# LemonATsu/UNet-PhaseGen

Measured on AMD Instinct MI355X. Metric: spectrogram-frames/sec (train fwd+bwd), higher is better.
Workload: dtype f32; 1 GPU; train.py full step (fwd + cos/sin/mag loss + bwd + Adam), UNetModel(1024, 2048), per-GPU batch 64 x 1024 bins x 256 frames (BASELINE configs[2]); global_batch=64, frames=256, channels=1024, parallelism=dp1, grad_allreduce_payload=fp32, adam=fused into the wgrad epilogues

## Files before the change

include/phasegen.h:

```cpp
#ifndef PHASEGEN_H
#define PHASEGEN_H
#include <stdint.h>

#ifdef __cplusplus
extern "C" {
#endif

#define PG_VERSION 400

enum { PG_OK = 0, PG_ERR_NULL = -1, PG_ERR_SHAPE = -2, PG_ERR_ALIGN = -3, PG_ERR_UNSUPPORTED = -4,
       PG_ERR_WORKSPACE = -5 };

enum { PG_ACT_NONE = 0, PG_ACT_LEAKY02 = 1 , PG_ACT_RELU = 2  };

struct pg_adam_args;
typedef struct pg_conv_args {
    int32_t B, Cin, Cout, Lin, Lout, k, stride, pad;
    const float* x;  int64_t x_bs;
    int32_t x_act;
    int32_t precision;
    const float* w;
    float* y;        int64_t y_bs;
    const float* dy; int64_t dy_bs;
    float* dx;       int64_t dx_bs;
    const float* dx_add; int64_t dx_add_bs;
    const float* dx_ref; int64_t dx_ref_bs;
    int32_t dx_mask;
    int32_t schedule;
    float* dw;
    int32_t y_act; int32_t y2_act;
    float* y2;       int64_t y2_bs;
    void* workspace; int64_t workspace_bytes;
    const struct pg_adam_args* adam;
} pg_conv_args;
int64_t pg_workspace_bytes_conv(void);
int64_t pg_workspace_bytes_wgrad(const pg_conv_args* a, int32_t op);
enum { PG_PREC_FP32 = 0, PG_PREC_BF16 = 1, PG_PREC_BF16X3 = 2 };
enum { PG_SCHED_AUTO = 0, PG_SCHED_TILE_PER_WG = 1, PG_SCHED_FORCE_STREAMK = 2, PG_SCHED_NO_RAW = 4, PG_SCHED_NO_TALL = 8,
       PG_SCHED_CONTENDED = 16, PG_SCHED_NO_PS = 128, PG_SCHED_NO_RAW3 = 0x2000, PG_SCHED_ALL_RAW3 = 0x4000, PG_SCHED_NO_COLSPLIT = 0x20000, PG_SCHED_COLSPLIT = 0x40000 };
#define PG_SCHED_OVERSUB(f) (((f) & 15) << 8)
#define PG_SCHED_SLOTS(n) (((n) & 31) << 19)

int pg_conv1d_fwd(const pg_conv_args* a, void* stream);
int pg_conv1d_dgrad(const pg_conv_args* a, void* stream);
int pg_conv1d_wgrad(const pg_conv_args* a, void* stream);
int pg_convt1d_fwd(const pg_conv_args* a, void* stream);
int pg_convt1d_dgrad(const pg_conv_args* a, void* stream);
int pg_convt1d_wgrad(const pg_conv_args* a, void* stream);
enum { PG_OP_CONV1D_FWD = 0, PG_OP_CONV1D_DGRAD = 1, PG_OP_CONV1D_WGRAD = 2,
       PG_OP_CONVT1D_FWD = 3, PG_OP_CONVT1D_DGRAD = 4, PG_OP_CONVT1D_WGRAD = 5 };
int pg_conv_describe(const pg_conv_args* a, int32_t op, char* buf, int32_t buflen);

#define PG_H_HEAD 32
typedef struct pg_convh_args {
// ... 238 lines not shown
```

unet-phasegen_amd/csrc/conv_common.h:

```cpp
#pragma once
#include <hip/hip_runtime.h>
#include <stdint.h>
#include "phasegen.h"
#include "pg_common.h"

namespace pgconv {

struct IgemmParams {
    const float* x; long x_bs;
    const float* w;
    const float* pt; long pt_bs;
    float* y; long y_bs;
    const float* add; long add_bs;
    const float* ref; long ref_bs;
    unsigned x_bytes, w_bytes, pt_bytes;
    int B, Q, M, Lx, Ly, k, s, p;
    int act_x, act_p, mask_mode;
    int U, u_off;
    int LP; float inv_LP;
    int a_vec;
    int tilesM, tilesN;
    int g_ps;
    int tn_stride;
    float* y2; long y2_bs; float y_slope, y2_slope;
// ... 439 lines not shown
constexpr int RS2 = 768, RS1 = 384;
constexpr int raw_gap(int tj) { return tj >= 8 ? 16 : tj; }
constexpr int RTILE_A = RBM * BK;
constexpr int g_wlp(int kw, int s) { return kw == 32 ? 64 : (kw == 8 ? (s == 1 ? 24 : 40) : 36); }

inline bool unet_ks(int k, int s) { return (k == 32 && s == 2) || (k == 8 && s == 1) || (k == 8 && s == 2) || (k == 4 && s == 2) || (k == 5 && s == 2); }

enum Kind { KIND_F, KIND_T, KIND_G };

}

namespace pgconv {
hipError_t launch_im2col(int kind, const IgemmParams& p, int grid, hipStream_t st, int prec);
hipError_t launch_raw_ft(int kind, const IgemmParams& p, int grid, hipStream_t st, int prec);
hipError_t launch_raw_ft_tall(int kind, const IgemmParams& p, int grid, hipStream_t st, int prec);
hipError_t launch_raw_g(const IgemmParams& p, int grid, hipStream_t st, int prec);
hipError_t launch_h3(int kind, const IgemmParams& p, int grid, hipStream_t st);
bool raw3_covers(int kind, const IgemmParams& p);
hipError_t launch_raw3(int kind, const IgemmParams& p, int grid, hipStream_t st);
bool h_supported(int kind, const IgemmParams& p);
}
```

unet-phasegen_amd/csrc/conv_igemm.hip:

```cpp
#include <hip/hip_runtime.h>
#include <cstring>
#include <cmath>
#include <algorithm>
#include "conv_fixup.h"

namespace {

constexpr int WG_PER_CU = 2;
constexpr int MAX_STREAMK_WG = 2048;
constexpr long WS_PER_WG = 2L * ACC_REGS * NT * 4;
constexpr long WS_STREAMK = (long)MAX_STREAMK_WG * WS_PER_WG;

struct Knobs {
    int prec;
    int force_mode;
    int no_raw;
    int no_tall;
    int oversub;
    int contended;
    int no_ps;
    int no_raw3;
    int all_raw3;
    int sr;
    int force_colsplit;
    int no_colsplit;
    int slots;
};
int decode_knobs(const pg_conv_args* a, Knobs& k) {
    if (a->precision < 0 || a->precision > 2) return pg_fail(PG_ERR_UNSUPPORTED, "conv: precision must be PG_PREC_FP32, PG_PREC_BF16 or PG_PREC_BF16X3");
    const int sc = a->schedule;
    if (sc < 0 || (sc & ~0xffffff) || ((sc >> 17) & 3) == 3 || (sc & 3) == 3 || ((sc >> 8) & 15) > 8) return pg_fail(PG_ERR_SHAPE, "conv: bad schedule bits");
    k.prec = a->precision;
    k.force_mode = sc & 3; k.no_raw = (sc >> 2) & 1; k.no_tall = (sc >> 3) & 1;
    k.oversub = (sc >> 8) & 15; if (!k.oversub) k.oversub = 4;
    k.contended = (sc >> 4) & 1;
    if ((sc >> 5) & 3) return pg_fail(PG_ERR_UNSUPPORTED, "conv: schedule bits 5-6 (tile families removed in 0.4)");
    k.no_ps = (sc >> 7) & 1;
    k.no_raw3 = (sc >> 13) & 1;
    k.all_raw3 = (sc >> 14) & 1;
    k.sr = ((sc >> 15) & 3) ? 1 << (((sc >> 15) & 3) - 1) : 0;
    k.no_colsplit = (sc >> 17) & 1;
    k.force_colsplit = (sc >> 18) & 1;
    k.slots = (sc >> 19) & 31;
    if (k.no_raw3 && k.all_raw3) return pg_fail(PG_ERR_SHAPE, "conv: schedule bits 13 and 14 exclude each other");
    return PG_OK;
}

bool fixup_wide(int grid, long split_tiles) { return split_tiles > 0 && grid >= 8 * split_tiles; }

int pick_grid(long tiles, int nslab, IgemmParams& p, long ws_bytes, const Knobs& kn, bool one_wave) {
    const long total = tiles * (long)nslab;
    const long slots = (long)(kn.slots ? kn.slots : pg_cu_count()) * (one_wave ? 1 : WG_PER_CU), ws_per_wg = one_wave ? 2 * WS_PER_WG : WS_PER_WG;
    ws_bytes = std::min(ws_bytes, WS_STREAMK);
    p.whole = 0;
    if (kn.force_mode == 0 && !kn.contended && tiles % slots == 0) {
        if (tiles <= slots * kn.oversub) return (int)tiles;
        for (long mult = kn.oversub; mult >= 1; --mult)
            if (tiles % (slots * mult) == 0) return (int)(slots * mult);
    }
// ... 39 lines not shown
    p.Kp = (int)kp; p.pk_bytes = (unsigned)pbytes;
    return (qbytes + 255) / 256 * 256 + pbytes;
}

enum Family { FAM_IM2COL, FAM_RAW, FAM_RAW_TALL, FAM_RAW3, FAM_G_RAW, FAM_G_PS, FAM_H3 };
enum Fixup { FIXUP_NONE, FIXUP_PLAIN, FIXUP_WIDE };
struct ConvPart {
    Family fam; int grid; long tiles; Fixup fixup;
    IgemmParams p;
};
struct ConvPlan {
    Kind kind; int prec;
    ConvPart main, tail;
    bool has_tail;
    long pack;
};

bool r3_ok(Kind kind, const IgemmParams& p, const Knobs& kn, long rows) {
    return kind != KIND_G && kn.prec == 0 && !kn.no_raw3 && raw_supported(kind, p, kn) && pgconv::raw3_covers(kind, p) &&
           (rows + 255) / 256 * 256 * 100 <= (rows + RBM - 1) / RBM * RBM * 103;
}

Family pick_family(Kind kind, const IgemmParams& p, const Knobs& kn, long rows, long cols) {
    const bool raw = raw_supported(kind, p, kn);
    if (kind == KIND_G) {
        if (!raw) return FAM_IM2COL;
        const long cps = (p.LP + 15) / 16;
        return p.k != 32 && (cps * 16 - p.LP) * 100 <= 7L * p.LP && !kn.no_ps ? FAM_G_PS : FAM_G_RAW;
    }
    const long cols_wide = (cols + RBN - 1) / RBN * RBN, cols_tall = (cols + RBN / 2 - 1) / (RBN / 2) * (RBN / 2);
// ... 92 lines not shown
    return PG_OK;
}

struct ConvOp { Kind kind; bool tr, swap; const char* null_msg; };
const ConvOp CONV_OPS[6] = {
    {KIND_F, false, false, "conv1d_fwd: x, w, y required"},
    {KIND_T, false, true, "conv1d_dgrad: dy, w, dx required"},
    {KIND_G, false, false, "conv1d_wgrad: dy, x, dw required"},
    {KIND_T, true, false, "convt1d_fwd: x, w, y required"},
    {KIND_F, true, true, "convt1d_dgrad: dy, w, dx required"},
    {KIND_G, true, true, "convt1d_wgrad: dy, x, dw required"}};

int plan_conv(int op, const pg_conv_args* a, bool ptrs, ConvPlan& pl) {
    const ConvOp& o = CONV_OPS[op];
    if (int e = check_geom(a, o.tr)) return e;
    Knobs kn; if (int e = decode_knobs(a, kn)) return e;
    IgemmParams p = {};
    p.B = a->B; p.k = a->k; p.s = a->stride; p.p = a->pad;
    p.M = o.swap ? a->Cin : a->Cout; p.Q = o.swap ? a->Cout : a->Cin; p.Lx = o.swap ? a->Lout : a->Lin;
    const int lo = o.swap ? a->Lin : a->Lout;
    p.x = o.swap ? a->dy : a->x; p.x_bs = o.swap ? a->dy_bs : a->x_bs; p.act_x = o.swap ? PG_ACT_NONE : a->x_act;
    if (o.kind == KIND_G) {
        p.pt = o.swap ? a->x : a->dy; p.pt_bs = o.swap ? a->x_bs : a->dy_bs; p.act_p = o.swap ? a->x_act : PG_ACT_NONE;
        p.LP = lo; p.y = a->dw;
    } else if (o.swap) {
        p.w = a->w; p.Ly = lo; p.y = a->dx; p.y_bs = a->dx_bs; p.y_slope = 1.0f; p.y2_slope = 1.0f;
        p.add = a->dx_add; p.add_bs = a->dx_add_bs; p.ref = a->dx_ref; p.ref_bs = a->dx_ref_bs;
        p.mask_mode = a->dx_ref ? a->dx_mask : 0;
    } else {
        p.w = a->w; p.Ly = lo; p.y = a->y; p.y_bs = a->y_bs; p.y_slope = pg_act_slope(a->y_act);
        p.y2 = a->y2; p.y2_bs = a->y2_bs; p.y2_slope = pg_act_slope(a->y2_act);
    }
    if (ptrs && (!p.x || !p.y || !(o.kind == KIND_G ? p.pt : p.w))) return pg_fail(PG_ERR_NULL, o.null_msg);
    long rows = p.M, cols = (long)p.B * p.Ly, K = (long)p.Q * p.k;
    if (o.kind == KIND_T) {
        p.u_off = p.p / p.s;
        p.U = (p.Ly - 1 + p.p) / p.s - p.u_off + 1;
        if (p.U <= 0) return pg_fail(PG_ERR_SHAPE, "convT: empty output");
        rows = (long)p.M * p.s; cols = (long)p.B * p.U; K = (long)p.Q * ((p.k + p.s - 1) / p.s);
    } else if (o.kind == KIND_G) {
        cols = (long)p.Q * p.k; K = (long)p.B * p.LP;
    }
    if (int e = set_extents(p)) return e;
    if (int e = o.kind == KIND_G ? set_fused_adam(p, a) : PG_OK) return e;
    p.ws = (float*)a->workspace;
    pl.kind = o.kind; pl.prec = kn.prec; pl.pack = 0;
    pl.has_tail = split_columns(o.kind, p, kn, rows, cols, K, a->workspace_bytes);
    if (pl.has_tail) {
        const long full = cols / RBN * RBN;
        if (int e = plan_part(FAM_RAW3, o.kind, kn, p, rows, 0, full, K, a->workspace_bytes, pl.main)) return e;
        return plan_part(FAM_RAW_TALL, o.kind, kn, p, rows, full, cols, K, a->workspace_bytes, pl.tail);
    }
    const Family fam = pick_family(o.kind, p, kn, rows, cols);
    if (int e = plan_part(fam, o.kind, kn, p, rows, 0, cols, K, a->workspace_bytes, pl.main)) return e;
    if ((pl.main.fam == FAM_G_RAW || pl.main.fam == FAM_G_PS) && kn.prec == 0 && (pl.pack = g_pack_layout(pl.main.p)) < 0)
        return pg_fail(PG_ERR_SHAPE, "wgrad: packed operand exceeds 2 GiB (31-bit buffer offsets)");
    return PG_OK;
}

int h3_params(const pg_convh_args* a, bool ptrs, IgemmParams& p, Knobs& kn) {
    if (!a) return pg_fail(PG_ERR_NULL, "conv_fwd_h: null args");
// ... 28 lines not shown
    if (tr) {
        p.u_off = p.p / p.s;
        p.U = (p.Ly - 1 + p.p) / p.s - p.u_off + 1;
        if (p.U <= 0) return pg_fail(PG_ERR_SHAPE, "conv_fwd_h: empty output");
    }
    if (!pgconv::h_supported(tr ? KIND_T : KIND_F, p)) return pg_fail(PG_ERR_UNSUPPORTED, "conv_fwd_h: geometry not covered by the bf16-resident kernels (use the fp32-tensor entry points)");
    return PG_OK;
}

int plan_h3(const pg_convh_args* a, ConvPlan& pl) {
    Knobs kn;
    ConvPart& c = pl.main;
    IgemmParams& p = c.p;
    if (int e = h3_params(a, true, p, kn)) return e;
    const bool tr = a->transposed != 0;
    pl.kind = tr ? KIND_T : KIND_F; pl.prec = 0; pl.has_tail = false; pl.pack = 0; c.fam = FAM_H3;
    const long rows = tr ? (long)p.M * p.s : p.M, cols = (long)p.B * (tr ? p.U : p.Ly);
    p.tilesM = (int)((rows + 255) / 256);
    p.tilesN = (int)((cols + 255) / 256);
    p.tn_stride = 256;
    p.nslab = (int)((long)p.Q * (tr ? pg_shadow_taps(p.k, p.s) : p.k) / 32);
    c.tiles = (long)p.tilesM * p.tilesN;
    if (c.tiles <= 0 || c.tiles > 0x0fffffffL || p.nslab <= 0) return pg_fail(PG_ERR_SHAPE, "conv_fwd_h: empty or oversize grid");
    set_grid(c, kn, a->workspace_bytes);
    return PG_OK;
}

hipError_t launch_fixup(const ConvPlan& pl, const ConvPart& c, hipStream_t st) {
    typedef void (*Fn)(const IgemmParams, int);
#define FIX2(KIND, MB, NB, WN) {conv_fixup_kernel<KIND, MB, NB, WN, false>, conv_fixup_kernel<KIND, MB, NB, WN, true>}
    static const Fn table[4][4][2] = {
// ... 17 lines not shown
    const Kind kind = pl.kind;
    const char* tk = kind == KIND_T ? "true" : "false";
    hipError_t e = hipSuccess;
    switch (c.fam) {
        case FAM_RAW_TALL:
            if (name) snprintf(name, 96, "conv_raw_kernel<%d, %d, %s, %d, 1>", p.k, p.s, tk, pl.prec);
            else e = pgconv::launch_raw_ft_tall(kind, p, c.grid, st, pl.prec);
            break;
        case FAM_RAW:
            if (name) snprintf(name, 96, "conv_raw_kernel<%d, %d, %s, %d, 2>", p.k, p.s, tk, pl.prec);
            else e = pgconv::launch_raw_ft(kind, p, c.grid, st, pl.prec);
            break;
        case FAM_G_RAW:
        case FAM_G_PS:
            if (name) snprintf(name, 96, "conv_g_%s_kernel<%d, %d, %d>", c.fam == FAM_G_PS ? "ps" : "raw", p.k, p.s, pl.prec);
            else e = pgconv::launch_raw_g(p, c.grid, st, pl.prec);
            break;
        case FAM_IM2COL:
            if (name) snprintf(name, 96, "conv_%c_kernel<0, 0, %d>", "ftg"[kind], pl.prec);
            else e = pgconv::launch_im2col(kind, p, c.grid, st, pl.prec);
            break;
        case FAM_RAW3:
            if (name) snprintf(name, 96, "conv_raw3_kernel<%d, %d, %s, %s>", p.k, p.s, tk, p.act_x == PG_ACT_NONE ? "false" : "true");
            else e = pgconv::launch_raw3(kind, p, c.grid, st);
            break;
        case FAM_H3:
            if (name) snprintf(name, 96, "conv_h3_kernel<%d, %d, %s>", kind == KIND_T && p.k == 5 ? 8 : p.k, p.s, tk);
            else e = pgconv::launch_h3(kind, p, c.grid, st);
            break;
    }
    if (!name && e == hipSuccess && c.fixup != FIXUP_NONE) e = launch_fixup(pl, c, st);
    return e;
}

void describe(const ConvPlan& pl, char* buf, int buflen) {
    static const char* const fixup_name[] = {"none", "plain", "wide"};
    const ConvPart& c = pl.main;
    char name[96];
    (void)part_kernel(pl, c, nullptr, name);
    snprintf(buf, (size_t)buflen, "%s|grid=%d|tiles=%ld|slabs=%d|split=%d|whole=%d|fixup=%s", name, c.grid, c.tiles, c.p.nslab,
             (int)(c.fixup != FIXUP_NONE), c.p.whole, fixup_name[c.fixup]);
    if (!pl.has_tail) return;
    (void)part_kernel(pl, pl.tail, nullptr, name);
    const size_t n = strlen(buf);
    if (n + 7 < (size_t)buflen) snprintf(buf + n, (size_t)buflen - n, "|tail=%s,grid=%d", name, pl.tail.grid);
}

int execute(ConvPlan& pl, long ws_bytes, hipStream_t st) {
    IgemmParams& p = pl.main.p;
    if (pl.pack) {
        if (!p.ws || ws_bytes < WS_STREAMK + pl.pack)
            return pg_fail(PG_ERR_WORKSPACE, "wgrad: the fp32 kernels need pg_workspace_bytes_wgrad() bytes of workspace (packed operands)");
        p.qk = reinterpret_cast<const float*>(reinterpret_cast<char*>(p.ws) + WS_STREAMK);
        p.pk = reinterpret_cast<const float*>(reinterpret_cast<const char*>(p.qk) + ((long)p.qk_bytes + 255) / 256 * 256);
    }
    hipError_t e = part_kernel(pl, pl.main, st);
    if (e == hipSuccess && pl.has_tail) e = part_kernel(pl, pl.tail, st);
    return e == hipSuccess ? PG_OK : pg_fail((int)e, hipGetErrorString(e));
}

int run_conv(int op, const pg_conv_args* a, void* stream) {
    ConvPlan pl;
    if (int e = plan_conv(op, a, true, pl)) return e;
    return execute(pl, a->workspace_bytes, (hipStream_t)stream);
}

}

extern "C" int pg_conv1d_fwd(const pg_conv_args* a, void* stream) { return run_conv(PG_OP_CONV1D_FWD, a, stream); }
// ... 43 lines not shown
```

unet-phasegen_amd/csrc/conv_raw_wgrad.hip:

```cpp
#include "conv_common.h"

namespace {

template <int KW, int S> struct GRaw {
    static constexpr int WL = 15 * S + KW;
    static constexpr int WLP = g_wlp(KW, S);
    static constexpr int NQT = RBN / KW;
    static constexpr int TNV = NQT * KW;
    static constexpr int SUB = NQT * WLP;
    static constexpr int SUBS = (SUB + 63) / 64 * 64;
    static constexpr int NE = (SUB + NT - 1) / NT;
    static constexpr int STG = RTILE_A + 2 * SUBS;
    static constexpr int SUBP = (SUB + 255) / 256 * 256;
    static_assert(WL <= WLP, "window does not fit its slot");
};

template <int KW, int S, int BF>
__device__ __forceinline__ void g_raw_bf(const IgemmParams& p) {
    using C = GRaw<KW, S>;
    __shared__ __attribute__((aligned(16))) float lds[2 * C::STG];
    const int tid = threadIdx.x, lane = tid & 63;
    const int wv = __builtin_amdgcn_readfirstlane(tid >> 6), wm = wv >> 1, wn = wv & 1;
    const int kt = dma_kt(lane, wv);
    const rsrc_t rp = make_rsrc(p.pt, p.pt_bytes), rx = make_rsrc(p.x, p.x_bytes);
// ... 568 lines not shown
        slot = 1;
    }
}

template <int KW, int S, int BF>
__global__ __launch_bounds__(NT, 2) void conv_g_raw_kernel(const IgemmParams p) {
    if constexpr (BF == 0) g_raw_f32<KW, S>(p);
    else g_raw_bf<KW, S, BF>(p);
}
template <int KW, int S, int BF>
__global__ __launch_bounds__(NT, 2) void conv_g_ps_kernel(const IgemmParams p) {
    if constexpr (BF == 0) g_ps_f32<KW, S>(p);
    else g_ps_bf<KW, S, BF>(p);
}

__global__ __launch_bounds__(256) void pack_rows_kernel(const float* __restrict__ src, long bs, int C, int L, int F, int W, unsigned n,
                                                       float slope, float* __restrict__ dst) {
    for (unsigned i = blockIdx.x * 256u + threadIdx.x; i < n; i += gridDim.x * 256u) {
        const unsigned r = i / (unsigned)W, b = r / (unsigned)C, c = r - b * (unsigned)C;
        const int t = (int)(i - r * (unsigned)W) - F;
        float v = 0.f;
        if ((unsigned)t < (unsigned)L) {
            v = src[(long)b * bs + (long)c * L + t];
            if (slope != 1.0f) v = pg_act_apply(v, slope);
        }
        dst[i] = v;
    }
}
__global__ __launch_bounds__(256) void pack_flat_kernel(const float* __restrict__ src, long bs, int B, int LP, int Kp, unsigned n,
                                                       float slope, float* __restrict__ dst) {
    for (unsigned i = blockIdx.x * 256u + threadIdx.x; i < n; i += gridDim.x * 256u) {
        const unsigned m = i / (unsigned)Kp, k = i - m * (unsigned)Kp, b = k / (unsigned)LP, t = k - b * (unsigned)LP;
        float v = 0.f;
        if ((int)b < B) {
            v = src[(long)b * bs + (long)m * LP + t];
            if (slope != 1.0f) v = pg_act_apply(v, slope);
        }
        dst[i] = v;
    }
}
unsigned pack_grid(unsigned n) { return (n + 255u) / 256u < 2048u ? (n + 255u) / 256u : 2048u; }

hipError_t pack_g(const IgemmParams& p, hipStream_t st) {
    float* const qk = const_cast<float*>(p.qk);
    float* const pk = const_cast<float*>(p.pk);
    const unsigned nq = (unsigned)(p.qk_bytes / 4), np = (unsigned)(p.pk_bytes / 4);
    hipLaunchKernelGGL(pack_rows_kernel, dim3(pack_grid(nq)), dim3(256), 0, st, p.x, p.x_bs, p.Q, p.Lx, p.p, p.Lq, nq, pg_act_slope(p.act_x), qk);
    if (p.g_ps) hipLaunchKernelGGL(pack_rows_kernel, dim3(pack_grid(np)), dim3(256), 0, st, p.pt, p.pt_bs, p.M, p.LP, 0, p.Kp, np, pg_act_slope(p.act_p), pk);
    else hipLaunchKernelGGL(pack_flat_kernel, dim3(pack_grid(np)), dim3(256), 0, st, p.pt, p.pt_bs, p.B, p.LP, p.Kp, np, pg_act_slope(p.act_p), pk);
    return hipGetLastError();
}

template <int KW, int S>
hipError_t launch_g_raw(const IgemmParams& p, int grid, hipStream_t st, int prec) {
    if (prec == 0) {
        if (hipError_t e = pack_g(p, st)) return e;
    }
    if (p.g_ps) {
        if (prec == 1) hipLaunchKernelGGL((conv_g_ps_kernel<KW, S, 1>), dim3(grid), dim3(NT), 0, st, p);
        else if (prec == 2) hipLaunchKernelGGL((conv_g_ps_kernel<KW, S, 2>), dim3(grid), dim3(NT), 0, st, p);
        else hipLaunchKernelGGL((conv_g_ps_kernel<KW, S, 0>), dim3(grid), dim3(NT), 0, st, p);
        return hipGetLastError();
    }
    if (prec == 1) hipLaunchKernelGGL((conv_g_raw_kernel<KW, S, 1>), dim3(grid), dim3(NT), 0, st, p);
    else if (prec == 2) hipLaunchKernelGGL((conv_g_raw_kernel<KW, S, 2>), dim3(grid), dim3(NT), 0, st, p);
    else hipLaunchKernelGGL((conv_g_raw_kernel<KW, S, 0>), dim3(grid), dim3(NT), 0, st, p);
    return hipGetLastError();
}

}

hipError_t pgconv::launch_raw_g(const IgemmParams& p, int grid, hipStream_t st, int prec) {
    if (p.k == 32) return launch_g_raw<32, 2>(p, grid, st, prec);
    if (p.k == 8 && p.s == 1) return launch_g_raw<8, 1>(p, grid, st, prec);
    if (p.k == 8) return launch_g_raw<8, 2>(p, grid, st, prec);
    if (p.k == 5) return launch_g_raw<5, 2>(p, grid, st, prec);
    return launch_g_raw<4, 2>(p, grid, st, prec);
}
```

unet-phasegen_amd/phasegen/_lib.py:

```python
import ctypes as C
import os

_HERE = os.path.dirname(os.path.abspath(__file__))
LIB_PATH = os.path.join(_HERE, "libphasegen.so")
ABI_VERSION = 400

ACT_NONE, ACT_LEAKY, ACT_RELU = 0, 1, 2
PREC_FP32, PREC_BF16, PREC_BF16X3 = 0, 1, 2
OK, ERR_NULL, ERR_SHAPE, ERR_ALIGN, ERR_UNSUPPORTED, ERR_WORKSPACE = 0, -1, -2, -3, -4, -5
OP_CONV1D_FWD, OP_CONV1D_DGRAD, OP_CONV1D_WGRAD, OP_CONVT1D_FWD, OP_CONVT1D_DGRAD, OP_CONVT1D_WGRAD = range(6)
SCHED_AUTO, SCHED_TILE_PER_WG, SCHED_FORCE_STREAMK, SCHED_NO_RAW, SCHED_NO_TALL, SCHED_CONTENDED = 0, 1, 2, 4, 8, 16
SCHED_NO_PS = 128
SCHED_NO_RAW3 = 0x2000
SCHED_ALL_RAW3 = 0x4000
SCHED_NO_COLSPLIT = 0x20000
SCHED_COLSPLIT = 0x40000


def SCHED_SLOTS(n):
    if not 0 <= n <= 31:
        raise ValueError("SCHED_SLOTS: n must be 0..31")
    return n << 19


RS_KAISER_BEST, RS_KAISER_FAST = 0, 1

c_float_p = C.c_void_p


class ConvArgs(C.Structure):
    _fields_ = [("B", C.c_int32), ("Cin", C.c_int32), ("Cout", C.c_int32), ("Lin", C.c_int32), ("Lout", C.c_int32),
# ... 259 lines not shown
```

unet-phasegen_amd/phasegen/ops.py:

```python
import contextlib
import ctypes as C
import threading

import torch

from . import _lib
from ._lib import ACT_LEAKY, ACT_NONE, ACT_RELU, SCHED_CONTENDED, SCHED_SLOTS, SCHED_TILE_PER_WG


def _stream():
    return C.c_void_p(torch.cuda.current_stream().cuda_stream)


def _on_current_device(t, name):
    if t.device.index != torch.cuda.current_device():
        raise ValueError(f"{name}: tensor is on {t.device} but the current device is cuda:{torch.cuda.current_device()} "
                         "(wrap the call in torch.cuda.device(...))")


class KernelTimer:

    def __init__(self):
        self.records = {}
        self.plans = {}
# ... 106 lines not shown
    def clear(self):
        self.d.clear()


_conv_ws = _StreamCache()
_caches = [_conv_ws]


def _workspace(cache, device, need, what):
    if need < 0:
        _lib.check(int(need), what)
    ws = cache.get(device, lambda: need, need)
    return ws.data_ptr(), ws.numel()


def conv_workspace(device):
    return _conv_ws.get(device, _lib.load().pg_workspace_bytes_conv)


def release_workspaces():
    for c in _caches:
        c.clear()


_PRECISIONS = {"fp32": 0, "f32": 0, "bf16": 1, "bf16x3": 2, 0: 0, 1: 1, 2: 2}


class _Defaults(threading.local):
    precision = 0
    schedule = 0
    stft_single = 0


_tls = _Defaults()


def precision_code(mode):
    if mode not in _PRECISIONS:
        raise ValueError(f"conv precision {mode!r}: expected fp32 / bf16 / bf16x3 (or 0 / 1 / 2)")
    return _PRECISIONS[mode]


def set_conv_precision(mode):
    _tls.precision = precision_code(mode)


def current_schedule():
    return _tls.schedule


def set_conv_schedule(mode):
    if mode < 0 or (mode & ~0xffe0ff) or (mode & 0x60000) == 0x60000 or (mode & 3) == 3 or (mode & 0x70) or (mode & 0x6000) == 0x6000:
        raise ValueError("conv schedule: bad mode")
    _tls.schedule = (_tls.schedule & 0xf00) | mode


def set_conv_oversubscribe(factor):
    if not 1 <= factor <= 8:
        raise ValueError("conv oversubscribe: factor must be 1..8")
# ... 77 lines not shown
    lib = _lib.load()
    _note_plan(a, _lib.OP_CONVT1D_DGRAD if transposed else _lib.OP_CONV1D_DGRAD)
    fn = lib.pg_convt1d_dgrad if transposed else lib.pg_conv1d_dgrad
    _lib.check(fn(C.byref(a), _stream()), "dgrad")
    return dx


def adam_args(p, m, v, step, lr=1e-3, beta1=0.9, beta2=0.999, eps=1e-8, grad_scale=1.0):
    a = _lib.AdamArgs()
    a.n = p.numel()
    a.p, a.m, a.v = _dense(p, "p"), _dense(m, "m"), _dense(v, "v")
    a.lr, a.beta1, a.beta2, a.eps, a.grad_scale, a.step = lr, beta1, beta2, eps, grad_scale, step
    return a


def conv_wgrad(x, dy, dw, stride, pad, x_act=ACT_NONE, transposed=False, precision=None, schedule=None, adam=None):
    Cin, Cout, k = _geom(transposed, dw.shape)
    B, _, Lin = x.shape
    a = _conv_args(transposed, B, Cin, Cout, Lin, k, stride, pad, x.device, precision, schedule)
    if tuple(x.shape) != (B, Cin, Lin) or tuple(dy.shape) != (B, Cout, a.Lout):
        raise ValueError(f"conv_wgrad: shapes x{tuple(x.shape)} dy{tuple(dy.shape)} dw{tuple(dw.shape)} inconsistent")
    a.x, a.x_bs = _act3(x, "x")
    a.dy, a.dy_bs = _act3(dy, "dy")
    a.dw = _dense(dw, "dw")
    a.x_act = x_act
    if adam is not None:
        if adam.n != dw.numel():
            raise ValueError("conv_wgrad: fused adam tensors must have dw's shape")
        a.adam = C.addressof(adam)
    lib = _lib.load()
    op = _lib.OP_CONVT1D_WGRAD if transposed else _lib.OP_CONV1D_WGRAD
    need = lib.pg_workspace_bytes_wgrad(C.byref(a), op)
    if need > a.workspace_bytes:
        ws = _conv_ws.get(x.device, lib.pg_workspace_bytes_conv, at_least=need)
        a.workspace, a.workspace_bytes = ws.data_ptr(), ws.numel()
    _note_plan(a, op)
    fn = lib.pg_convt1d_wgrad if transposed else lib.pg_conv1d_wgrad
    _lib.check(fn(C.byref(a), _stream()), "wgrad")
    return dw


H_HEAD = 32
H_TAIL = 40


def h_pitch(L):
    return (L + H_TAIL + 7) // 8 * 8
# ... 766 lines not shown
```

unet-phasegen_amd/phasegen/unet.py:

```python
import math

import numpy as np
import torch

from . import detgen, ops
from .ops import ACT_LEAKY, ACT_NONE, ACT_RELU

ALIGN = 64

LAYERS = {
    "D0": (detgen.K_D0, "c", 2, 16), "D1": (detgen.K_D1, "c", 1, 2), "D2": (detgen.K_D2, "c", 2, 1),
    "D3": (detgen.K_D3, "c", 2, 1), "U3": (detgen.K_U3, "t", 2, 1), "U2": (detgen.K_U2, "t", 2, 1),
    "U1": (detgen.K_U1, "t", 1, 2), "U0": (detgen.K_U0, "t", 2, 16),
}
BN_OF = {"D1": detgen.BN_D1, "D2": detgen.BN_D2, "U3": detgen.BN_U3, "U2": detgen.BN_U2, "U1": detgen.BN_U1,
         "U0": detgen.BN_U0}
BACKWARD_ORDER = ["U0", "U1", "U2", "U3", "D3", "D2", "D1", "D0"]

CONTENDED_DGRAD = {"U0": ops.SCHED_CONTENDED, "U1": ops.SCHED_CONTENDED, "U2": ops.SCHED_CONTENDED, "U3": 0,
                   "D3": 0, "D2": ops.SCHED_CONTENDED, "D1": ops.SCHED_CONTENDED}
CONTENDED_WGRAD = {name: ops.SCHED_TILE_PER_WG for name in BACKWARD_ORDER}


def frame_plan(L):
# ... 74 lines not shown
                self.buffers[k].copy_(torch.as_tensor(np.asarray(params[k])))


class UNetEngine:

    def __init__(self, C, device=None, precision=None):
        if not torch.cuda.is_available():
            raise RuntimeError("phasegen.UNetEngine needs an MI355X (no CPU fallback exists for the hot path)")
        self.C = C
        self.device = torch.device("cuda", torch.cuda.current_device()) if device is None else torch.device(device)
        if self.device.index is None:
            self.device = torch.device("cuda", torch.cuda.current_device())
        self.precision = None if precision is None else ops.precision_code(precision)
        self.graphs = False
        self.contended = False
        self.fwd_count = 0
        self.arena = ParamArena(C, self.device)
        self.plans = {}
        self.bn_save = {k: (torch.empty(2 * C, device=self.device), torch.empty(2 * C, device=self.device))
                        for k in BN_OF}
        self.cur = None

    def plan(self, B, L):
        key = (B, L)
        if key not in self.plans:
            C = self.C
            L1, L2, L3, L4 = frame_plan(L)
            dev = self.device

            def z(*s):
# ... 210 lines not shown
        f = plan["fwd"]
        B = x0.shape[0]
        g = self._bwd_bufs(plan, B)
        a = self.arena
        h = 2 * self.C
        g_out = g_out.contiguous()
        def sched(table, name):
            return (ops.current_schedule() | table[name]) if self.contended else None

        def bn_bwd(name, raw, dy, dx):
            key = BN_OF[name]
            sm, si = self.bn_save[name]
            with ops.timed("hbm:bn_bwd." + name, 12 * raw.numel()):
                ops.bn_bwd(raw, dy, dx, a.p(key + ".weight"), sm, si, a.g(key + ".weight"), a.g(key + ".bias"))

        def wgrad(name, x, dy, act):
            key, kind, s, p = LAYERS[name]
            adam = fused_adam(key) if fused_adam is not None else None
            with ops.timed(name + ".wgrad"):
                ops.conv_wgrad(x, dy, a.g(key), s, p, x_act=act, transposed=(kind == "t"), precision=self.precision,
                               schedule=sched(CONTENDED_WGRAD, name), adam=adam)

        def dgrad(name, dy, dx, **kw):
            key, kind, s, p = LAYERS[name]
            with ops.timed(name + ".dgrad"):
                ops.conv_dgrad(dy, a.p(key), dx, s, p, transposed=(kind == "t"), precision=self.precision,
                               schedule=sched(CONTENDED_DGRAD, name), **kw)

        def ready(name):
            if on_grads_ready is not None:
                on_grads_ready(name)

        def done(name):
            if on_layer_done is not None:
                on_layer_done(name)

        def layer(name, wg, dg=None, **dkw):
            if fused_adam is None:
                wgrad(name, *wg)
                ready(name)
                if dg is not None:
                    dgrad(name, *dg, **dkw)
            else:
                if dg is not None:
                    dgrad(name, *dg, **dkw)
                wgrad(name, *wg)
                ready(name)
            done(name)

        for name, cat, raw, gin, g_raw, g_cat in (("U0", "cat0", "r0", g_out, "g_r0", "g_cat0"),
                                                  ("U1", "cat1", "r1", g["g_cat0"][:, h:], "g_r1", "g_cat1"),
                                                  ("U2", "cat2", "r2", g["g_cat1"][:, h:], "g_r2", "g_cat2"),
                                                  ("U3", "d3", "r3", g["g_cat2"][:, h:], "g_r3", "g_d3")):
            bn_bwd(name, f[raw], gin, g[g_raw])
            layer(name, (f[cat], g[g_raw], ACT_NONE), (g[g_raw], g[g_cat]), ref=f[cat], mask=ACT_RELU)
        layer("D3", (f["l2"], g["g_d3"], ACT_NONE), (g["g_d3"], g["g_cat2"][:, :h]), add=g["g_cat2"][:, :h], ref=f["l2"], mask=ACT_LEAKY)
        bn_bwd("D2", f["c2"], g["g_cat2"][:, :h], g["g_c2"])
        layer("D2", (f["l1"], g["g_c2"], ACT_NONE), (g["g_c2"], g["g_cat1"][:, :h]), add=g["g_cat1"][:, :h], ref=f["l1"], mask=ACT_LEAKY)
        bn_bwd("D1", f["c1"], g["g_cat1"][:, :h], g["g_c1"])
        layer("D1", (f["l0"], g["g_c1"], ACT_NONE), (g["g_c1"], g["g_cat0"][:, :h]), add=g["g_cat0"][:, :h], ref=f["l0"], mask=ACT_LEAKY)
        layer("D0", (x0, g["g_cat0"][:, :h], ACT_NONE))
# ... 16 lines not shown
```

Before: 99020 frames/s.

## Split fp32 wgrad operand packing into a stage that can overlap dgrad on a side stream

Replaces the separate scalar pack_rows/pack_flat kernels with one fused pack kernel that handles both operands with one wave per row unit and 16-byte vector loads and stores. Adds schedule bits to run only the pack or only the GEMM of the fp32 wgrad, plus an opt-in UNet path that packs on a side stream while dgrad runs, synchronised with events. The aim is to cut pack launch and bandwidth overhead and to hide packing behind dgrad. In exchange, the overlap needs a shared workspace sized for the largest layer, and the two streams now compete for bandwidth.

```diff
diff --git a/include/phasegen.h b/include/phasegen.h
--- a/include/phasegen.h
+++ b/include/phasegen.h
@@ -37,7 +37,8 @@
 int64_t pg_workspace_bytes_wgrad(const pg_conv_args* a, int32_t op);
 enum { PG_PREC_FP32 = 0, PG_PREC_BF16 = 1, PG_PREC_BF16X3 = 2 };
 enum { PG_SCHED_AUTO = 0, PG_SCHED_TILE_PER_WG = 1, PG_SCHED_FORCE_STREAMK = 2, PG_SCHED_NO_RAW = 4, PG_SCHED_NO_TALL = 8,
-       PG_SCHED_CONTENDED = 16, PG_SCHED_NO_PS = 128, PG_SCHED_NO_RAW3 = 0x2000, PG_SCHED_ALL_RAW3 = 0x4000, PG_SCHED_NO_COLSPLIT = 0x20000, PG_SCHED_COLSPLIT = 0x40000 };
+       PG_SCHED_CONTENDED = 16, PG_SCHED_NO_PS = 128, PG_SCHED_NO_RAW3 = 0x2000, PG_SCHED_ALL_RAW3 = 0x4000, PG_SCHED_NO_COLSPLIT = 0x20000, PG_SCHED_COLSPLIT = 0x40000,
+       PG_SCHED_PACK_ONLY = 0x1000000, PG_SCHED_PACKED = 0x2000000 };
 #define PG_SCHED_OVERSUB(f) (((f) & 15) << 8)
 #define PG_SCHED_SLOTS(n) (((n) & 31) << 19)
 
diff --git a/unet-phasegen_amd/csrc/conv_common.h b/unet-phasegen_amd/csrc/conv_common.h
--- a/unet-phasegen_amd/csrc/conv_common.h
+++ b/unet-phasegen_amd/csrc/conv_common.h
@@ -477,7 +477,8 @@
 hipError_t launch_im2col(int kind, const IgemmParams& p, int grid, hipStream_t st, int prec);
 hipError_t launch_raw_ft(int kind, const IgemmParams& p, int grid, hipStream_t st, int prec);
 hipError_t launch_raw_ft_tall(int kind, const IgemmParams& p, int grid, hipStream_t st, int prec);
-hipError_t launch_raw_g(const IgemmParams& p, int grid, hipStream_t st, int prec);
+enum { PACK_BOTH = 0, PACK_ONLY = 1, PACK_CALLER = 2 };
+hipError_t launch_raw_g(const IgemmParams& p, int grid, hipStream_t st, int prec, int pack_mode);
 hipError_t launch_h3(int kind, const IgemmParams& p, int grid, hipStream_t st);
 bool raw3_covers(int kind, const IgemmParams& p);
 hipError_t launch_raw3(int kind, const IgemmParams& p, int grid, hipStream_t st);
diff --git a/unet-phasegen_amd/csrc/conv_igemm.hip b/unet-phasegen_amd/csrc/conv_igemm.hip
--- a/unet-phasegen_amd/csrc/conv_igemm.hip
+++ b/unet-phasegen_amd/csrc/conv_igemm.hip
@@ -25,11 +25,12 @@
     int force_colsplit;
     int no_colsplit;
     int slots;
+    int pack_mode;
 };
-int decode_knobs(const pg_conv_args* a, Knobs& k) {
+int decode_knobs(const pg_conv_args* a, Knobs& k, bool wgrad = false) {
     if (a->precision < 0 || a->precision > 2) return pg_fail(PG_ERR_UNSUPPORTED, "conv: precision must be PG_PREC_FP32, PG_PREC_BF16 or PG_PREC_BF16X3");
     const int sc = a->schedule;
-    if (sc < 0 || (sc & ~0xffffff) || ((sc >> 17) & 3) == 3 || (sc & 3) == 3 || ((sc >> 8) & 15) > 8) return pg_fail(PG_ERR_SHAPE, "conv: bad schedule bits");
+    if (sc < 0 || (sc & ~(wgrad ? 0x3ffffff : 0xffffff)) || ((sc >> 17) & 3) == 3 || (sc & 3) == 3 || ((sc >> 8) & 15) > 8) return pg_fail(PG_ERR_SHAPE, "conv: bad schedule bits");
     k.prec = a->precision;
     k.force_mode = sc & 3; k.no_raw = (sc >> 2) & 1; k.no_tall = (sc >> 3) & 1;
     k.oversub = (sc >> 8) & 15; if (!k.oversub) k.oversub = 4;
@@ -43,6 +44,8 @@
     k.force_colsplit = (sc >> 18) & 1;
     k.slots = (sc >> 19) & 31;
     if (k.no_raw3 && k.all_raw3) return pg_fail(PG_ERR_SHAPE, "conv: schedule bits 13 and 14 exclude each other");
+    if ((sc & PG_SCHED_PACK_ONLY) && (sc & PG_SCHED_PACKED)) return pg_fail(PG_ERR_UNSUPPORTED, "conv: PG_SCHED_PACK_ONLY and PG_SCHED_PACKED exclude each other");
+    k.pack_mode = (sc & PG_SCHED_PACK_ONLY) ? pgconv::PACK_ONLY : ((sc & PG_SCHED_PACKED) ? pgconv::PACK_CALLER : pgconv::PACK_BOTH);
     return PG_OK;
 }
 
@@ -112,6 +115,7 @@
     ConvPart main, tail;
     bool has_tail;
     long pack;
+    int pack_mode;
 };
 
 bool r3_ok(Kind kind, const IgemmParams& p, const Knobs& kn, long rows) {
@@ -234,7 +238,7 @@
 int plan_conv(int op, const pg_conv_args* a, bool ptrs, ConvPlan& pl) {
     const ConvOp& o = CONV_OPS[op];
     if (int e = check_geom(a, o.tr)) return e;
-    Knobs kn; if (int e = decode_knobs(a, kn)) return e;
+    Knobs kn; if (int e = decode_knobs(a, kn, o.kind == KIND_G)) return e;
     IgemmParams p = {};
     p.B = a->B; p.k = a->k; p.s = a->stride; p.p = a->pad;
     p.M = o.swap ? a->Cin : a->Cout; p.Q = o.swap ? a->Cout : a->Cin; p.Lx = o.swap ? a->Lout : a->Lin;
@@ -265,6 +269,7 @@
     if (int e = o.kind == KIND_G ? set_fused_adam(p, a) : PG_OK) return e;
     p.ws = (float*)a->workspace;
     pl.kind = o.kind; pl.prec = kn.prec; pl.pack = 0;
+    pl.pack_mode = o.kind == KIND_G ? kn.pack_mode : pgconv::PACK_BOTH;
     pl.has_tail = split_columns(o.kind, p, kn, rows, cols, K, a->workspace_bytes);
     if (pl.has_tail) {
         const long full = cols / RBN * RBN;
@@ -323,7 +328,7 @@
     IgemmParams& p = c.p;
     if (int e = h3_params(a, true, p, kn)) return e;
     const bool tr = a->transposed != 0;
-    pl.kind = tr ? KIND_T : KIND_F; pl.prec = 0; pl.has_tail = false; pl.pack = 0; c.fam = FAM_H3;
+    pl.kind = tr ? KIND_T : KIND_F; pl.prec = 0; pl.has_tail = false; pl.pack = 0; pl.pack_mode = pgconv::PACK_BOTH; c.fam = FAM_H3;
     const long rows = tr ? (long)p.M * p.s : p.M, cols = (long)p.B * (tr ? p.U : p.Ly);
     p.tilesM = (int)((rows + 255) / 256);
     p.tilesN = (int)((cols + 255) / 256);
@@ -371,7 +376,7 @@
         case FAM_G_RAW:
         case FAM_G_PS:
             if (name) snprintf(name, 96, "conv_g_%s_kernel<%d, %d, %d>", c.fam == FAM_G_PS ? "ps" : "raw", p.k, p.s, pl.prec);
-            else e = pgconv::launch_raw_g(p, c.grid, st, pl.prec);
+            else e = pgconv::launch_raw_g(p, c.grid, st, pl.prec, pl.pack_mode);
             break;
         case FAM_IM2COL:
             if (name) snprintf(name, 96, "conv_%c_kernel<0, 0, %d>", "ftg"[kind], pl.prec);
@@ -397,6 +402,10 @@
     (void)part_kernel(pl, c, nullptr, name);
     snprintf(buf, (size_t)buflen, "%s|grid=%d|tiles=%ld|slabs=%d|split=%d|whole=%d|fixup=%s", name, c.grid, c.tiles, c.p.nslab,
              (int)(c.fixup != FIXUP_NONE), c.p.whole, fixup_name[c.fixup]);
+    if (pl.pack_mode != pgconv::PACK_BOTH) {
+        const size_t n = strlen(buf);
+        if (n + 13 < (size_t)buflen) snprintf(buf + n, (size_t)buflen - n, "|pack=%s", pl.pack_mode == pgconv::PACK_ONLY ? "only" : "caller");
+    }
     if (!pl.has_tail) return;
     (void)part_kernel(pl, pl.tail, nullptr, name);
     const size_t n = strlen(buf);
@@ -405,11 +414,16 @@
 
 int execute(ConvPlan& pl, long ws_bytes, hipStream_t st) {
     IgemmParams& p = pl.main.p;
+    if (pl.pack_mode == pgconv::PACK_ONLY && !pl.pack) return PG_OK;
     if (pl.pack) {
         if (!p.ws || ws_bytes < WS_STREAMK + pl.pack)
             return pg_fail(PG_ERR_WORKSPACE, "wgrad: the fp32 kernels need pg_workspace_bytes_wgrad() bytes of workspace (packed operands)");
         p.qk = reinterpret_cast<const float*>(reinterpret_cast<char*>(p.ws) + WS_STREAMK);
         p.pk = reinterpret_cast<const float*>(reinterpret_cast<const char*>(p.qk) + ((long)p.qk_bytes + 255) / 256 * 256);
+    }
+    if (pl.pack_mode == pgconv::PACK_ONLY) {
+        const hipError_t e = pgconv::launch_raw_g(p, 0, st, pl.prec, pl.pack_mode);
+        return e == hipSuccess ? PG_OK : pg_fail((int)e, hipGetErrorString(e));
     }
     hipError_t e = part_kernel(pl, pl.main, st);
     if (e == hipSuccess && pl.has_tail) e = part_kernel(pl, pl.tail, st);
diff --git a/unet-phasegen_amd/csrc/conv_raw_wgrad.hip b/unet-phasegen_amd/csrc/conv_raw_wgrad.hip
--- a/unet-phasegen_amd/csrc/conv_raw_wgrad.hip
+++ b/unet-phasegen_amd/csrc/conv_raw_wgrad.hip
@@ -606,48 +606,119 @@
     else g_ps_bf<KW, S, BF>(p);
 }
 
-__global__ __launch_bounds__(256) void pack_rows_kernel(const float* __restrict__ src, long bs, int C, int L, int F, int W, unsigned n,
-                                                       float slope, float* __restrict__ dst) {
-    for (unsigned i = blockIdx.x * 256u + threadIdx.x; i < n; i += gridDim.x * 256u) {
-        const unsigned r = i / (unsigned)W, b = r / (unsigned)C, c = r - b * (unsigned)C;
-        const int t = (int)(i - r * (unsigned)W) - F;
-        float v = 0.f;
-        if ((unsigned)t < (unsigned)L) {
-            v = src[(long)b * bs + (long)c * L + t];
-            if (slope != 1.0f) v = pg_act_apply(v, slope);
-        }
-        dst[i] = v;
-    }
-}
-__global__ __launch_bounds__(256) void pack_flat_kernel(const float* __restrict__ src, long bs, int B, int LP, int Kp, unsigned n,
-                                                       float slope, float* __restrict__ dst) {
-    for (unsigned i = blockIdx.x * 256u + threadIdx.x; i < n; i += gridDim.x * 256u) {
-        const unsigned m = i / (unsigned)Kp, k = i - m * (unsigned)Kp, b = k / (unsigned)LP, t = k - b * (unsigned)LP;
-        float v = 0.f;
-        if ((int)b < B) {
-            v = src[(long)b * bs + (long)m * LP + t];
-            if (slope != 1.0f) v = pg_act_apply(v, slope);
-        }
-        dst[i] = v;
-    }
-}
-unsigned pack_grid(unsigned n) { return (n + 255u) / 256u < 2048u ? (n + 255u) / 256u : 2048u; }
+struct PackRows {
+    const float* src; float* dst; long bs; int nrow, C, L, F, W, rw, segs; float inv_nch, slope;
+};
+struct PackFlat {
+    const float* src; float* dst; long bs; int M, B, LP, Kp, rw, segs; float inv_nch, inv_LP, slope;
+};
+struct PackUnit {
+    int r0, nr, ch0, n;
+    __device__ __forceinline__ PackUnit(unsigned u, int rows, int nch, int rw, int segs) {
+        if (segs > 1) { r0 = (int)(u / (unsigned)segs); nr = 1; ch0 = ((int)u - r0 * segs) * 256; n = min(256, nch - ch0); }
+        else { r0 = (int)u * rw; nr = min(rw, rows - r0); ch0 = 0; n = nch; }
+    }
+    __device__ __forceinline__ void piece(int idx, int nch, float inv_nch, int& q, int& ch) const {
+        if (nr == 1) { q = 0; ch = ch0 + idx; }
+        else divmod24(idx, nch, inv_nch, q, ch);
+    }
+};
+__device__ __forceinline__ f32x4 pack_load4(const float* __restrict__ sp, int t, int L) {
+    f32x4 v = {0.f, 0.f, 0.f, 0.f};
+    if (t >= 0 && t + 4 <= L) {
+        __builtin_memcpy(&v, sp + t, 16);
+    } else {
+#pragma unroll
+        for (int e = 0; e < 4; ++e)
+            if ((unsigned)(t + e) < (unsigned)L) v[e] = sp[t + e];
+    }
+    return v;
+}
+__device__ __forceinline__ void pack_store4(float* __restrict__ dp, f32x4 v, float slope) {
+    if (slope != 1.0f) {
+#pragma unroll
+        for (int e = 0; e < 4; ++e) v[e] = pg_act_apply(v[e], slope);
+    }
+    *reinterpret_cast<f32x4*>(dp) = v;
+}
+__device__ __forceinline__ void pack_rows(const PackRows& o, unsigned gw, unsigned nw, int lane) {
+    const int nch = o.W >> 2;
+    const unsigned nunits = o.segs > 1 ? (unsigned)o.nrow * o.segs : ((unsigned)o.nrow + o.rw - 1) / o.rw;
+    for (unsigned u = gw; u < nunits; u += nw) {
+        const PackUnit un(u, o.nrow, nch, o.rw, o.segs);
+        const int b0 = un.r0 / o.C, c0 = un.r0 - b0 * o.C;
+        for (int idx = lane; idx < un.nr * un.n; idx += 64) {
+            int q, ch;
+            un.piece(idx, nch, o.inv_nch, q, ch);
+            int b = b0, c = c0 + q;
+            if (c >= o.C) { c -= o.C; ++b; }
+            const float* const sp = o.src + (long)b * o.bs + (long)c * o.L;
+            pack_store4(o.dst + (long)(un.r0 + q) * o.W + 4 * ch, pack_load4(sp, 4 * ch - o.F, o.L), o.slope);
+        }
+    }
+}
+__device__ __forceinline__ void pack_flat(const PackFlat& o, unsigned gw, unsigned nw, int lane) {
+    const int nch = o.Kp >> 2, K = o.B * o.LP;
+    const unsigned nunits = o.segs > 1 ? (unsigned)o.M * o.segs : ((unsigned)o.M + o.rw - 1) / o.rw;
+    for (unsigned u = gw; u < nunits; u += nw) {
+        const PackUnit un(u, o.M, nch, o.rw, o.segs);
+        for (int idx = lane; idx < un.nr * un.n; idx += 64) {
+            int q, ch;
+            un.piece(idx, nch, o.inv_nch, q, ch);
+            const int m = un.r0 + q, k0 = 4 * ch;
+            f32x4 v = {0.f, 0.f, 0.f, 0.f};
+            if (k0 < K) {
+                int b, i0;
+                if (K < (1 << 24)) divmod24(k0, o.LP, o.inv_LP, b, i0);
+                else { b = k0 / o.LP; i0 = k0 - b * o.LP; }
+                const float* const sp = o.src + (long)b * o.bs + (long)m * o.LP;
+                v = pack_load4(sp, i0, o.LP);
+                if (i0 + 4 > o.LP && b + 1 < o.B) {
+                    const float* const sn = sp + o.bs;
+#pragma unroll
+                    for (int e = 1; e < 4; ++e)
+                        if (i0 + e >= o.LP) v[e] = sn[i0 + e - o.LP];
+                }
+            }
+            pack_store4(o.dst + (long)m * o.Kp + k0, v, o.slope);
+        }
+    }
+}
+__global__ __launch_bounds__(256) void pack_g_kernel(const PackRows q, const PackRows pr, const PackFlat pf) {
+    const int lane = threadIdx.x & 63;
+    const unsigned gw = blockIdx.x * 4u + (threadIdx.x >> 6), nw = gridDim.x * 4u;
+    pack_rows(q, gw, nw, lane);
+    if (pr.nrow) pack_rows(pr, gw, nw, lane);
+    if (pf.M) pack_flat(pf, gw, nw, lane);
+}
+void pack_units(int nch, int cap, int& rw, int& segs, long& units, long rows) {
+    segs = nch > 256 ? (nch + 255) / 256 : 1;
+    rw = segs > 1 ? 1 : std::max(1, std::min(std::min(256 / nch, 64), cap));
+    units = segs > 1 ? rows * segs : (rows + rw - 1) / rw;
+}
 
 hipError_t pack_g(const IgemmParams& p, hipStream_t st) {
     float* const qk = const_cast<float*>(p.qk);
     float* const pk = const_cast<float*>(p.pk);
-    const unsigned nq = (unsigned)(p.qk_bytes / 4), np = (unsigned)(p.pk_bytes / 4);
-    hipLaunchKernelGGL(pack_rows_kernel, dim3(pack_grid(nq)), dim3(256), 0, st, p.x, p.x_bs, p.Q, p.Lx, p.p, p.Lq, nq, pg_act_slope(p.act_x), qk);
-    if (p.g_ps) hipLaunchKernelGGL(pack_rows_kernel, dim3(pack_grid(np)), dim3(256), 0, st, p.pt, p.pt_bs, p.M, p.LP, 0, p.Kp, np, pg_act_slope(p.act_p), pk);
-    else hipLaunchKernelGGL(pack_flat_kernel, dim3(pack_grid(np)), dim3(256), 0, st, p.pt, p.pt_bs, p.B, p.LP, p.Kp, np, pg_act_slope(p.act_p), pk);
+    PackRows q = {p.x, qk, p.x_bs, p.B * p.Q, p.Q, p.Lx, p.p, p.Lq, 1, 1, 4.0f / (float)p.Lq, pg_act_slope(p.act_x)};
+    PackRows pr = {};
+    PackFlat pf = {};
+    long uq, up;
+    pack_units(p.Lq / 4, p.Q, q.rw, q.segs, uq, q.nrow);
+    if (p.g_ps) {
+        pr = {p.pt, pk, p.pt_bs, p.B * p.M, p.M, p.LP, 0, p.Kp, 1, 1, 4.0f / (float)p.Kp, pg_act_slope(p.act_p)};
+        pack_units(p.Kp / 4, p.M, pr.rw, pr.segs, up, pr.nrow);
+    } else {
+        pf = {p.pt, pk, p.pt_bs, p.M, p.B, p.LP, p.Kp, 1, 1, 4.0f / (float)p.Kp, 1.0f / (float)p.LP, pg_act_slope(p.act_p)};
+        pack_units(p.Kp / 4, p.M, pf.rw, pf.segs, up, pf.M);
+    }
+    const long wg = (std::max(uq, up) + 3) / 4;
+    hipLaunchKernelGGL(pack_g_kernel, dim3((unsigned)std::min(wg, 2048L)), dim3(256), 0, st, q, pr, pf);
     return hipGetLastError();
 }
 
 template <int KW, int S>
 hipError_t launch_g_raw(const IgemmParams& p, int grid, hipStream_t st, int prec) {
-    if (prec == 0) {
-        if (hipError_t e = pack_g(p, st)) return e;
-    }
     if (p.g_ps) {
         if (prec == 1) hipLaunchKernelGGL((conv_g_ps_kernel<KW, S, 1>), dim3(grid), dim3(NT), 0, st, p);
         else if (prec == 2) hipLaunchKernelGGL((conv_g_ps_kernel<KW, S, 2>), dim3(grid), dim3(NT), 0, st, p);
@@ -662,7 +733,11 @@
 
 }
 
-hipError_t pgconv::launch_raw_g(const IgemmParams& p, int grid, hipStream_t st, int prec) {
+hipError_t pgconv::launch_raw_g(const IgemmParams& p, int grid, hipStream_t st, int prec, int pack_mode) {
+    if (prec == 0 && pack_mode != PACK_CALLER) {
+        if (hipError_t e = pack_g(p, st)) return e;
+    }
+    if (pack_mode == PACK_ONLY) return hipSuccess;
     if (p.k == 32) return launch_g_raw<32, 2>(p, grid, st, prec);
     if (p.k == 8 && p.s == 1) return launch_g_raw<8, 1>(p, grid, st, prec);
     if (p.k == 8) return launch_g_raw<8, 2>(p, grid, st, prec);
diff --git a/unet-phasegen_amd/phasegen/_lib.py b/unet-phasegen_amd/phasegen/_lib.py
--- a/unet-phasegen_amd/phasegen/_lib.py
+++ b/unet-phasegen_amd/phasegen/_lib.py
@@ -15,6 +15,8 @@
 SCHED_ALL_RAW3 = 0x4000
 SCHED_NO_COLSPLIT = 0x20000
 SCHED_COLSPLIT = 0x40000
+SCHED_PACK_ONLY = 0x1000000
+SCHED_PACKED = 0x2000000
 
 
 def SCHED_SLOTS(n):
diff --git a/unet-phasegen_amd/phasegen/ops.py b/unet-phasegen_amd/phasegen/ops.py
--- a/unet-phasegen_amd/phasegen/ops.py
+++ b/unet-phasegen_amd/phasegen/ops.py
@@ -5,7 +5,7 @@
 import torch
 
 from . import _lib
-from ._lib import ACT_LEAKY, ACT_NONE, ACT_RELU, SCHED_CONTENDED, SCHED_SLOTS, SCHED_TILE_PER_WG
+from ._lib import ACT_LEAKY, ACT_NONE, ACT_RELU, SCHED_CONTENDED, SCHED_PACK_ONLY, SCHED_PACKED, SCHED_SLOTS, SCHED_TILE_PER_WG
 
 
 def _stream():
@@ -144,8 +144,8 @@
     return ws.data_ptr(), ws.numel()
 
 
-def conv_workspace(device):
-    return _conv_ws.get(device, _lib.load().pg_workspace_bytes_conv)
+def conv_workspace(device, at_least=0):
+    return _conv_ws.get(device, _lib.load().pg_workspace_bytes_conv, at_least=at_least)
 
 
 def release_workspaces():
@@ -173,6 +173,10 @@
 
 def set_conv_precision(mode):
     _tls.precision = precision_code(mode)
+
+
+def current_precision():
+    return _tls.precision
 
 
 def current_schedule():
@@ -280,10 +284,28 @@
     return a
 
 
-def conv_wgrad(x, dy, dw, stride, pad, x_act=ACT_NONE, transposed=False, precision=None, schedule=None, adam=None):
+_WGRAD_STAGES = {None: 0, "pack": _lib.SCHED_PACK_ONLY, "gemm": _lib.SCHED_PACKED}
+
+
+def wgrad_workspace_bytes(x, dw, stride, pad, transposed=False, precision=None, schedule=None):
+    Cin, Cout, k = _geom(transposed, dw.shape)
+    a = _conv_args(transposed, x.shape[0], Cin, Cout, x.shape[2], k, stride, pad, None, precision, schedule)
+    need = _lib.load().pg_workspace_bytes_wgrad(C.byref(a), _lib.OP_CONVT1D_WGRAD if transposed else _lib.OP_CONV1D_WGRAD)
+    if need < 0:
+        _lib.check(int(need), "workspace_bytes_wgrad")
+    return need
+
+
+def conv_wgrad(x, dy, dw, stride, pad, x_act=ACT_NONE, transposed=False, precision=None, schedule=None, adam=None, stage=None,
+               workspace=None):
+    if stage not in _WGRAD_STAGES:
+        raise ValueError(f"conv_wgrad: stage {stage!r}: expected None, 'pack' or 'gemm'")
     Cin, Cout, k = _geom(transposed, dw.shape)
     B, _, Lin = x.shape
-    a = _conv_args(transposed, B, Cin, Cout, Lin, k, stride, pad, x.device, precision, schedule)
+    a = _conv_args(transposed, B, Cin, Cout, Lin, k, stride, pad, x.device if workspace is None else None, precision, schedule)
+    a.schedule |= _WGRAD_STAGES[stage]
+    if workspace is not None:
+        a.workspace, a.workspace_bytes = _dense_as(workspace, torch.uint8, "workspace"), workspace.numel()
     if tuple(x.shape) != (B, Cin, Lin) or tuple(dy.shape) != (B, Cout, a.Lout):
         raise ValueError(f"conv_wgrad: shapes x{tuple(x.shape)} dy{tuple(dy.shape)} dw{tuple(dw.shape)} inconsistent")
     a.x, a.x_bs = _act3(x, "x")
@@ -296,7 +318,7 @@
         a.adam = C.addressof(adam)
     lib = _lib.load()
     op = _lib.OP_CONVT1D_WGRAD if transposed else _lib.OP_CONV1D_WGRAD
-    need = lib.pg_workspace_bytes_wgrad(C.byref(a), op)
+    need = lib.pg_workspace_bytes_wgrad(C.byref(a), op) if workspace is None else 0
     if need > a.workspace_bytes:
         ws = _conv_ws.get(x.device, lib.pg_workspace_bytes_conv, at_least=need)
         a.workspace, a.workspace_bytes = ws.data_ptr(), ws.numel()
diff --git a/unet-phasegen_amd/phasegen/unet.py b/unet-phasegen_amd/phasegen/unet.py
--- a/unet-phasegen_amd/phasegen/unet.py
+++ b/unet-phasegen_amd/phasegen/unet.py
@@ -112,6 +112,9 @@
         self.precision = None if precision is None else ops.precision_code(precision)
         self.graphs = False
         self.contended = False
+        self.overlap_pack = False
+        self._pack_stream = None
+        self._pack_events = {}
         self.fwd_count = 0
         self.arena = ParamArena(C, self.device)
         self.plans = {}
@@ -352,12 +355,39 @@
             with ops.timed("hbm:bn_bwd." + name, 12 * raw.numel()):
                 ops.bn_bwd(raw, dy, dx, a.p(key + ".weight"), sm, si, a.g(key + ".weight"), a.g(key + ".bias"))
 
-        def wgrad(name, x, dy, act):
+        def wgrad(name, x, dy, act, stage=None, workspace=None):
             key, kind, s, p = LAYERS[name]
-            adam = fused_adam(key) if fused_adam is not None else None
+            adam = fused_adam(key) if fused_adam is not None and stage != "pack" else None
             with ops.timed(name + ".wgrad"):
                 ops.conv_wgrad(x, dy, a.g(key), s, p, x_act=act, transposed=(kind == "t"), precision=self.precision,
-                               schedule=sched(CONTENDED_WGRAD, name), adam=adam)
+                               schedule=sched(CONTENDED_WGRAD, name), adam=adam, stage=stage, workspace=workspace)
+
+        pack_ws = None
+        if (fused_adam is not None and self.overlap_pack and ops._timer is None
+                and (ops.current_precision() if self.precision is None else self.precision) == 0):
+            if "wgrad_ws" not in plan:
+                plan["wgrad_ws"] = max(
+                    ops.wgrad_workspace_bytes(x, a.g(LAYERS[n][0]), LAYERS[n][2], LAYERS[n][3], transposed=(LAYERS[n][1] == "t"),
+                                              precision=self.precision)
+                    for n, x in (("U0", f["cat0"]), ("U1", f["cat1"]), ("U2", f["cat2"]), ("U3", f["d3"]), ("D3", f["l2"]),
+                                 ("D2", f["l1"]), ("D1", f["l0"])))
+            pack_ws = ops.conv_workspace(self.device, at_least=plan["wgrad_ws"])
+            if self._pack_stream is None:
+                self._pack_stream = torch.cuda.Stream(self.device)
+            main, side = torch.cuda.current_stream(self.device), self._pack_stream
+
+        def packed_wgrad(name, wg, dg, dkw):
+            if name not in self._pack_events:
+                self._pack_events[name] = (torch.cuda.Event(), torch.cuda.Event())
+            ready_ev, packed_ev = self._pack_events[name]
+            ready_ev.record(main)
+            with torch.cuda.stream(side):
+                side.wait_event(ready_ev)
+                wgrad(name, *wg, stage="pack", workspace=pack_ws)
+                packed_ev.record(side)
+            dgrad(name, *dg, **dkw)
+            main.wait_event(packed_ev)
+            wgrad(name, *wg, stage="gemm", workspace=pack_ws)
 
         def dgrad(name, dy, dx, **kw):
             key, kind, s, p = LAYERS[name]
@@ -380,9 +410,12 @@
                 if dg is not None:
                     dgrad(name, *dg, **dkw)
             else:
-                if dg is not None:
-                    dgrad(name, *dg, **dkw)
-                wgrad(name, *wg)
+                if dg is not None and pack_ws is not None:
+                    packed_wgrad(name, wg, dg, dkw)
+                else:
+                    if dg is not None:
+                        dgrad(name, *dg, **dkw)
+                    wgrad(name, *wg)
                 ready(name)
             done(name)
 
```

After: 99100 frames/s (median of 2 runs). No clear change (+0.1%).
